# yanxian-ll/GS-SR

Measured on AMD Instinct MI355X. Metric: train iters/sec @300k Gaussians 1080p (rasterize fwd+bwd ms and HBM GB/s vs roofline alongside), higher is better.
Workload: dtype f32; 1 GPU; diff_surfel_rasterization forward+backward (2DGS surfel: the rasterizer of configs[1] scaffold-2dgs) + fused L1/linear image loss + fused Adam (gsrast.optim, one HIP kernel) on EXPLICIT Gaussians, colors_precomp, P=300000, 1920x1080, synthetic scene SURVEY §8d (seed=rank); the complete methods (decode, SSIM, regularisers, statistics) are timed in method_iteration (--full); variant=surfel, P=300000, W=1920, H=1080, parallelism=1 independent tile(s), 1 per GPU, no collective

## Files before the change

gs-sr_amd/csrc/gsr_api.hip:

```cpp
#include "gsr_common.h"
#include <atomic>
#include <cstdarg>
#include <cstdio>
#include <cstring>
#include <mutex>

int gsr_tile_sort_passes(int T);

static thread_local char g_err[512] = "";
void gsr_set_error(const char* fmt, ...)
{
    va_list ap;
    va_start(ap, fmt);
    vsnprintf(g_err, sizeof(g_err), fmt, ap);
    va_end(ap);
}
extern "C" const char* gsr_last_error(void) { return g_err; }
extern "C" int32_t gsr_abi_version(void) { return GSR_ABI_VERSION; }

int gsr_check_launch(const char* what, hipStream_t s, bool debug)
{
    hipError_t e = hipGetLastError();
    if (e != hipSuccess) { gsr_set_error("%s: launch failed: %s", what, hipGetErrorString(e)); return 1; }
    if (debug) {
// ... 54 lines not shown
        else { (void)hipEventCreate(&r.a); (void)hipEventCreate(&r.b); }
        r.label = label;
        (void)hipEventRecord(r.a, s);
    }
    ~ProfScope()
    {
        if (!on) return;
        (void)hipEventRecord(r.b, s);
        std::lock_guard<std::mutex> lk(g_prof_mu);
        g_prof.push_back(r);
    }
};
extern "C" int gsr_profile_enable(int32_t enable)
{
    std::lock_guard<std::mutex> lk(g_prof_mu);
    prof_drain();
    const uint32_t mask = ((uint32_t)enable >> 8) & 0xFFu;
    g_prof_on = enable == 0 ? 0u : ((enable == 1 || mask == 0u) ? 0xFFu : mask);
    for (int i = 0; i < GSR_PROF_LABELS; i++) { g_prof_ms[i] = 0; g_prof_n[i] = 0; }
    return 0;
}
extern "C" int gsr_profile_read(double* ms_total, uint64_t* counts)
{
    std::lock_guard<std::mutex> lk(g_prof_mu);
    prof_drain();
    for (int i = 0; i < GSR_PROF_LABELS; i++) { ms_total[i] = g_prof_ms[i]; counts[i] = g_prof_n[i]; }
    return 0;
}

template <typename T>
static T* take(char*& p, size_t n)
{
    T* r = reinterpret_cast<T*>(p);
    p += gsr_align(n * sizeof(T));
    return r;
}

GeomView gsr_carve_geom(int variant, int P, void* base)
{
    GeomView g;
    char* p = reinterpret_cast<char*>(base);
    const size_t n = (size_t)(P > 0 ? P : 1);
    const uint32_t nblk = gsr_div_up((uint32_t)n, GSR_SORT_BLOCK);
    g.depth_key = take<uint32_t>(p, n);
    g.tiles_touched = take<uint32_t>(p, n);
    g.rect = take<ushort4>(p, n);
    g.cull = take<float4>(p, n * 2);
    g.rec = take<float4>(p, n * gsr_rec_stride(variant));
    g.clamped = take<uint32_t>(p, n);
    g.vals_a = take<uint32_t>(p, n);
    g.offsets = take<uint32_t>(p, n);
    g.keys_b = take<uint32_t>(p, n);
    g.vals_b = take<uint32_t>(p, n);
    g.sorted_idx = g.vals_a;
    g.hist = take<uint32_t>(p, gsr_sort_hist_words(nblk, 256));
    g.scan_tmp = take<uint32_t>(p, gsr_div_up((uint32_t)n, 256) + 64);
    g.counters = take<uint32_t>(p, 64);
    g.bytes = (size_t)(p - reinterpret_cast<char*>(base));
    return g;
}

BinView gsr_carve_bin(int variant, uint32_t R, int W, int H, void* base)
{
    (void)variant;
    BinView b;
    char* p = reinterpret_cast<char*>(base);
    const size_t n = R > 0 ? R : 1;
    const uint32_t nblk = gsr_div_up((uint32_t)n, GSR_SORT_BLOCK);
    b.point_list = take<uint32_t>(p, n);
    b.tile_keys = take<uint32_t>(p, n);
    b.keys_b = take<uint32_t>(p, n);
    b.vals_b = take<uint32_t>(p, n);
    b.hist = take<uint32_t>(p, gsr_sort_hist_words(nblk, 256));
    b.scan_tmp = take<uint32_t>(p, 64);
    {
        const size_t T = (size_t)((W + GSR_TILE - 1) / GSR_TILE) * ((H + GSR_TILE - 1) / GSR_TILE);
        b.qmask = take<unsigned long long>(p, ((n >> 6) + T + 2) * 4);
        b.tile_tab = take<uint32_t>(p, gsr_tile_bucket_words((uint32_t)n, T) + (T <= (size_t)GSR_TB_TILES_MAX ? (size_t)GSR_TB_ROWS_MAX * GSR_TB_GROUPS_MAX : (size_t)2));
    }
    b.cap = R;
    b.bytes = (size_t)(p - reinterpret_cast<char*>(base));
    return b;
}

ImgView gsr_carve_img(int variant, int W, int H, void* base)
{
    ImgView im;
    char* p = reinterpret_cast<char*>(base);
    const size_t N = (size_t)W * H;
    const int gx = (W + GSR_TILE - 1) / GSR_TILE, gy = (H + GSR_TILE - 1) / GSR_TILE;
    im.final_T = take<float>(p, N * (variant == GSR_SURFEL ? 3 : 1));
    im.n_contrib = take<uint32_t>(p, N * (variant == GSR_SURFEL ? 2 : 1));
    im.ranges = take<uint2>(p, (size_t)gx * gy);
    im.tile_order = take<uint32_t>(p, (size_t)gx * gy + 1);
    im.bytes = (size_t)(p - reinterpret_cast<char*>(base));
    return im;
}

extern "C" size_t gsr_geom_bytes(int32_t variant, int32_t P) { return gsr_carve_geom(variant, P, nullptr).bytes; }
extern "C" size_t gsr_img_bytes(int32_t variant, int32_t W, int32_t H) { return gsr_carve_img(variant, W, H, nullptr).bytes; }
extern "C" size_t gsr_binning_bytes(int32_t variant, uint32_t R, int32_t W, int32_t H) { return gsr_carve_bin(variant, R, W, H, nullptr).bytes; }
extern "C" size_t gsr_backward_scratch_bytes(int32_t variant, int32_t P)
{
    return gsr_align((size_t)(P > 0 ? P : 1) * gsr_acc_stride(variant) * sizeof(float));
}

// ... 85 lines not shown
        if (!forced && mb->global_ttl.load(std::memory_order_relaxed) > 0) global = true;
    }
    return global;
}
uint32_t* gsr_long_list_word()
{
    Mailbox* mb = mailbox();
    return mb ? mb->dev + 16 * GSR_MAIL_SLOTS : nullptr;
}

const uint32_t* gsr_static_tile_map(int gx, int gy, hipStream_t s)
{
    struct Ent { int dev, gx, gy; uint32_t* map; };
    static std::mutex mu;
    static std::vector<Ent> cache;
    int dev = 0;
    if (hipGetDevice(&dev) != hipSuccess) return nullptr;
    std::lock_guard<std::mutex> lk(mu);
    for (const Ent& e : cache) if (e.dev == dev && e.gx == gx && e.gy == gy) return e.map;
    {
        hipStreamCaptureStatus cs = hipStreamCaptureStatusNone;
        if (hipStreamIsCapturing(s, &cs) != hipSuccess || cs != hipStreamCaptureStatusNone) { (void)hipGetLastError(); return nullptr; }
    }
    const int T = gx * gy, B = 4, bxn = (gx + B - 1) / B, byn = (gy + B - 1) / B;
    std::vector<std::vector<uint32_t>> lists(8);
    for (int by = 0; by < byn; by++)
        for (int bx = 0; bx < bxn; bx++) {
            std::vector<uint32_t>& L = lists[(bx + 3 * by) & 7];
            for (int ty = by * B; ty < std::min(gy, by * B + B); ty++)
                for (int tx = bx * B; tx < std::min(gx, bx * B + B); tx++) L.push_back((uint32_t)(ty * gx + tx));
        }
    std::vector<uint32_t> map((size_t)T);
    size_t pos[8] = {0, 0, 0, 0, 0, 0, 0, 0};
    for (int b = 0; b < T; b++) {
        int x = b & 7;
        for (int k = 0; k < 8 && pos[x] >= lists[x].size(); k++) x = (x + 1) & 7;
        map[(size_t)b] = lists[x][pos[x]++];
    }
    uint32_t* d = nullptr;
    if (hipMalloc(&d, (size_t)T * sizeof(uint32_t)) != hipSuccess) { (void)hipGetLastError(); return nullptr; }
    if (hipMemcpy(d, map.data(), (size_t)T * sizeof(uint32_t), hipMemcpyHostToDevice) != hipSuccess) { (void)hipGetLastError(); (void)hipFree(d); return nullptr; }
    cache.push_back({dev, gx, gy, d});
    return d;
}

#define GSR_PREFILTERED_MSG "Point is filtered although prefiltered is set. This shouldn't happen!"

static int check_cull_agreement(const gsr_cfg* cfg, const GeomView& g, hipStream_t s)
{
    if (!cfg->debug) return 0;
    uint32_t w = 0u;
    GSR_CHECK(hipMemcpyAsync(&w, g.counters + GSR_CNT_CULL_MISMATCH, sizeof(uint32_t), hipMemcpyDeviceToHost, s), "read cull agreement word");
    GSR_CHECK(hipStreamSynchronize(s), "debug sync");
    if (w) { gsr_set_error("tile culling: k_duplicate emitted a different number of instances than the preprocess kernel counted (gsr_tile_cull.h evaluated differently in the two units)"); return 1; }
    return 0;
}

extern "C" int gsr_forward_stage1_ex(const gsr_cfg* cfg, const gsr_inputs* in, void* geom, size_t geom_bytes,
                                     int32_t* radii, uint32_t* num_rendered_host, uint32_t* depth_order_host, void* stream)
{
    if (check_cfg(cfg, in)) return 1;
    hipStream_t s = (hipStream_t)stream;
    *num_rendered_host = 0;
    if (depth_order_host) *depth_order_host = 0u;
    if (cfg->P == 0) return 0;
    GeomView g = gsr_carve_geom(cfg->variant, cfg->P, geom);
    if (g.bytes > geom_bytes) { gsr_set_error("geom buffer too small: %zu < %zu", geom_bytes, g.bytes); return 1; }
    Mailbox* mb = mailbox();
    const unsigned slot = mb ? take_slot(mb) : 0u;
    struct SlotGuard { Mailbox* m; unsigned s; ~SlotGuard() { if (m) release_slot(m, s); } } guard{mb, slot};
    if (mb) mb->host[16 * slot + 1] = 0u;
    const bool global_order = gsr_decide_depth_order(cfg);
    if (depth_order_host) *depth_order_host = global_order ? GSR_MODE_GLOBAL : GSR_MODE_TILE;
    { ProfScope ps(GSR_PROF_PREPROCESS, s); if (gsr_launch_preprocess(cfg, in, g, radii, s, global_order, mb ? mb->dev + 16 * slot + 1 : nullptr)) return 1; }
    { ProfScope ps(GSR_PROF_DEPTH_ORDER, s); if (gsr_launch_depth_order(cfg, g, mb ? mb->dev + 16 * slot : nullptr, s, global_order, true)) return 1; }
    if (mb) {
        GSR_CHECK(hipStreamSynchronize(s), "stage1 sync");
        *num_rendered_host = *(volatile uint32_t*)(mb->host + 16 * slot);
        if (cfg->prefiltered && *(volatile uint32_t*)(mb->host + 16 * slot + 1)) { gsr_set_error("%s", GSR_PREFILTERED_MSG); return 1; }
    } else {
        GSR_CHECK(hipMemcpyAsync(num_rendered_host, g.counters, sizeof(uint32_t), hipMemcpyDeviceToHost, s), "read num_rendered");
        GSR_CHECK(hipStreamSynchronize(s), "stage1 sync");
    }
    return 0;
}
extern "C" int gsr_forward_stage1(const gsr_cfg* cfg, const gsr_inputs* in, void* geom, size_t geom_bytes,
                                  int32_t* radii, uint32_t* num_rendered_host, void* stream)
{
    return gsr_forward_stage1_ex(cfg, in, geom, geom_bytes, radii, num_rendered_host, nullptr, stream);
}

extern "C" int gsr_forward_stage2_ex(const gsr_cfg* cfg, const gsr_inputs* in, void* geom, size_t geom_bytes,
                                     void* binning, size_t binning_bytes, void* img, size_t img_bytes,
                                     uint32_t num_rendered, uint32_t depth_order, const gsr_outputs* out, void* stream)
{
    if (check_cfg(cfg, in)) return 1;
    hipStream_t s = (hipStream_t)stream;
    (void)geom_bytes;
    GeomView g = gsr_carve_geom(cfg->variant, cfg->P, geom);
    const uint32_t cap = gsr_binning_capacity(cfg->variant, binning_bytes, cfg->W, cfg->H);
    if (cap < num_rendered) { gsr_set_error("binning buffer too small: holds %u instances, need %u", cap, num_rendered); return 1; }
    BinView b = gsr_carve_bin(cfg->variant, cap, cfg->W, cfg->H, binning);
    ImgView im = gsr_carve_img(cfg->variant, cfg->W, cfg->H, img);
    if (im.bytes > img_bytes) { gsr_set_error("img buffer too small: %zu < %zu", img_bytes, im.bytes); return 1; }
    if (cfg->P == 0) {
        return 0;
    }
// ... 199 lines not shown
```

gs-sr_amd/csrc/gsr_binning.hip:

```cpp
#include "gsr_common.h"
#include "gsr_tile_sort.h"
#include "gsr_tile_cull.h"
#include <cstdlib>

__device__ __forceinline__ uint32_t lane_id() { return __builtin_amdgcn_mbcnt_hi(~0u, __builtin_amdgcn_mbcnt_lo(~0u, 0u)); }
__device__ __forceinline__ uint64_t lanemask_lt() { return (1ull << lane_id()) - 1ull; }

__device__ __forceinline__ uint32_t wave_incl_scan(uint32_t v)
{
#pragma unroll
    for (int d = 1; d < 64; d <<= 1) {
        uint32_t t = __shfl_up(v, d, 64);
        if ((int)lane_id() >= d) v += t;
    }
    return v;
}

__device__ __forceinline__ uint32_t block_incl_scan(uint32_t v, uint32_t* lds , uint32_t* total)
{
    const uint32_t lane = threadIdx.x & 63, wave = threadIdx.x >> 6, nw = (blockDim.x + 63) >> 6;
    uint32_t s = wave_incl_scan(v);
    if (lane == 63) lds[wave] = s;
    __syncthreads();
    if (wave == 0) {
// ... 251 lines not shown
        if (dm) hipLaunchKernelGGL(k_scan_rows, dim3(mask + 1), dim3(256), 0, s, H, nblk, gh);
        if (big_blocks) hipLaunchKernelGGL((k_radix_scatter<16, 256>), g, b, 0, s, kin, vin, kout, vout, n, n_dev, shift, bits, H, gh, ngroups, gh_next, dm);
        else hipLaunchKernelGGL((k_radix_scatter<GSR_SORT_ITEMS, 256>), g, b, 0, s, kin, vin, kout, vout, n, n_dev, shift, bits, H, gh, ngroups, gh_next, dm);
        uint32_t* t;
        t = kin; kin = kout; kout = t;
        if (vin == nullptr) { vin = vout; vout = vals_a; }
        else { t = vin; vin = vout; vout = t; }
        in_b = !in_b;
        shift += bits;
    }
    if (result_in_b) *result_in_b = in_b;
    return 0;
}


__global__ void __launch_bounds__(GSR_SCAN_BLOCK) k_offsets_local(const uint32_t* __restrict__ sorted_idx, const uint32_t* __restrict__ tiles_touched,
                                                                  uint32_t P, uint32_t* __restrict__ offsets, uint32_t* __restrict__ block_sums)
{
    __shared__ uint32_t lds[17];
    const uint32_t i = blockIdx.x * GSR_SCAN_BLOCK + threadIdx.x;
    uint32_t v = (i < P) ? tiles_touched[sorted_idx ? sorted_idx[i] : i] : 0;
    uint32_t tot;
    uint32_t incl = block_incl_scan(v, lds, &tot);
    if (i < P) offsets[i] = incl;
    if (threadIdx.x == 0) block_sums[blockIdx.x] = tot;
}
bool gsr_depth_order_static_rule(int P, int T, bool* forced, int variant)
{
    static int mode = -1;
    if (mode < 0) { const char* e = getenv("GSR_DEPTH_ORDER"); mode = !e ? 0 : (e[0] == 'g' ? 1 : (e[0] == 't' ? 2 : 0)); }
    if (forced) *forced = mode != 0;
    if (mode == 1) return true;
    if (mode == 2) return false;
    const long long per_tile = variant == GSR_EWA ? 155ll : (variant == GSR_PLANE ? 176ll : 192ll);
    return (long long)P > per_tile * (long long)T;
}

int gsr_launch_depth_order(const gsr_cfg* cfg, GeomView g, uint32_t* host_word_dev, hipStream_t s, bool global_order, bool need_total)
{
    const uint32_t P = (uint32_t)cfg->P;
    if (!global_order) {
        if (need_total)
            hipLaunchKernelGGL(k_scan_small, dim3(1), dim3(GSR_SCAN_BLOCK), 0, s, g.scan_tmp, gsr_div_up(P, 256u), g.counters, host_word_dev, 1);
        return gsr_check_launch("depth_order", s, cfg->debug);
    }
    bool in_b = false;
    if (gsr_radix_sort_pairs(g.depth_key, g.vals_a, g.keys_b, g.vals_b, P, nullptr, 0, 32, 8, true, g.hist, &in_b, s, false, true)) return 1;
    const uint32_t nblk = gsr_div_up(P, GSR_SCAN_BLOCK);
    hipLaunchKernelGGL(k_offsets_local, dim3(nblk), dim3(GSR_SCAN_BLOCK), 0, s, g.sorted_idx, g.tiles_touched, P, g.offsets, g.scan_tmp);
    hipLaunchKernelGGL(k_scan_small, dim3(1), dim3(GSR_SCAN_BLOCK), 0, s, g.scan_tmp, nblk, g.counters, host_word_dev);
    return gsr_check_launch("depth_order", s, cfg->debug);
}

template <int CULLV>
__global__ void __launch_bounds__(256) k_duplicate(uint32_t P, const uint32_t* __restrict__ sorted_idx, const uint32_t* __restrict__ offsets,
                                                   const uint32_t* __restrict__ block_prefix, const uint32_t* __restrict__ tiles_touched,
                                                   const ushort4* __restrict__ rect, const float4* __restrict__ cull, int gx,
                                                   uint32_t* __restrict__ keys, uint32_t* __restrict__ vals, uint32_t cap,
                                                   uint2* __restrict__ ranges, uint32_t T, uint32_t* __restrict__ zero_ptr, uint32_t zero_n,
                                                   uint32_t* __restrict__ order_valid, uint32_t scan_block,
                                                   uint32_t self_nblk, uint32_t* __restrict__ total_out, uint32_t* __restrict__ host_word)
{
    const uint32_t lane = threadIdx.x & 63u;
    const uint32_t i = (blockIdx.x * blockDim.x + threadIdx.x);
    if (i < T) ranges[i] = make_uint2(0xFFFFFFFFu, 0u);
    for (uint32_t z = i; z < zero_n; z += gridDim.x * blockDim.x) zero_ptr[z] = 0u;
    if (i == 0) *order_valid = 0u;
    const bool v = i < P;
    const uint32_t g = v ? (sorted_idx ? sorted_idx[i] : i) : 0u;
    const uint32_t cnt = v ? tiles_touched[g] : 0u;
    uint32_t bp = 0u;
    if (self_nblk) {
        __shared__ uint32_t s_red[4];
        if (blockIdx.x < self_nblk) {
            uint32_t part = 0u;
            for (uint32_t j = threadIdx.x; j < blockIdx.x; j += 256u) part += block_prefix[j];
#pragma unroll
            for (int d = 32; d >= 1; d >>= 1) part += (uint32_t)__shfl_xor((int)part, d, 64);
            if (lane == 0) s_red[threadIdx.x >> 6] = part;
            __syncthreads();
            bp = (s_red[0] + s_red[1]) + (s_red[2] + s_red[3]);
            if (blockIdx.x == self_nblk - 1u && threadIdx.x == 0) {
                const uint32_t tot = bp + block_prefix[blockIdx.x];
                *total_out = tot;
                if (host_word) __hip_atomic_store(host_word, tot, __ATOMIC_RELAXED, __HIP_MEMORY_SCOPE_SYSTEM);
            }
        }
    } else if (v) bp = block_prefix[i / scan_block];
    const uint32_t incl = v ? offsets[i] + bp : 0u;
    ushort4 r = make_ushort4(0, 0, 1, 1);
    if (cnt) r = rect[g];
    const uint32_t wave_base = __shfl(incl - cnt, 0, 64);
    if constexpr (CULLV >= 0) {
        __shared__ float4 s_cull[2 * 256];
        __shared__ float2 s_slope[256];
        __shared__ ushort4 s_rect[256];
        const uint32_t wbase = threadIdx.x & ~63u;
        float4 c0 = make_float4(0.f, 0.f, 0.f, 0.f), c1 = make_float4(0.f, -1.f, 0.f, 0.f);
        if (cnt) { c0 = cull[2 * (size_t)g]; c1 = cull[2 * (size_t)g + 1]; }
        s_cull[2 * threadIdx.x] = c0; s_cull[2 * threadIdx.x + 1] = c1; s_slope[threadIdx.x] = tc_slopes(c0, c1); s_rect[threadIdx.x] = r;
        __builtin_amdgcn_fence(__ATOMIC_ACQ_REL, "wavefront");
        __builtin_amdgcn_wave_barrier();
        const uint32_t area = cnt ? ((uint32_t)r.z - (uint32_t)r.x) * ((uint32_t)r.w - (uint32_t)r.y) : 0u;
        const uint32_t ai = wave_incl_scan(area);
        const uint32_t total = (uint32_t)__shfl((int)ai, 63, 64), excl = ai - area;
        uint32_t run = wave_base;
        for (uint32_t k0 = 0; k0 < total; k0 += 64u) {
            const TcCand c = tc_candidate<CULLV>(k0 + lane, total, excl, s_cull + 2 * wbase, s_slope + wbase, s_rect + wbase);
            const uint64_t hits = __ballot(c.hit);
            const uint32_t off = run + (uint32_t)__popcll(hits & lanemask_lt());
            const uint32_t sg = (uint32_t)__shfl((int)g, (int)c.s, 64);
            if (c.hit && off < cap) {
                keys[off] = c.ty * (uint32_t)gx + c.tx;
                vals[off] = sg;
            }
            run += (uint32_t)__popcll(hits);
        }
        const uint32_t counted = (uint32_t)__shfl((int)wave_incl_scan(cnt), 63, 64);
        if (lane == 0 && run - wave_base != counted) total_out[GSR_CNT_CULL_MISMATCH] = 1u;
        return;
    }
    uint32_t last = __shfl(incl, 63, 64);
    {
        const uint64_t vm = __ballot(v);
        if (vm != ~0ull) last = vm ? __shfl(incl, 63 - __builtin_clzll(vm), 64) : wave_base;
    }
    const uint32_t total = last - wave_base;
    const uint32_t excl = v ? (incl - cnt) - wave_base : total;
    const uint32_t w = (uint32_t)r.z - (uint32_t)r.x;
    const float rw = 1.0f / (float)(w ? w : 1u);
    for (uint32_t k0 = 0; k0 < total; k0 += 64u) {
        const uint32_t k = k0 + lane;
        uint32_t s = 0;
#pragma unroll
        for (uint32_t step = 32; step >= 1; step >>= 1) {
            const uint32_t t = s + step;
            const uint32_t e = __shfl(excl, t & 63u, 64);
            if (t < 64u && e <= k) s = t;
        }
        const uint32_t j = k - __shfl(excl, s, 64);
        const uint32_t sw = __shfl(w, s, 64), sx0 = __shfl((uint32_t)r.x, s, 64), sy0 = __shfl((uint32_t)r.y, s, 64), sg = __shfl(g, s, 64);
        const float srw = __shfl(rw, s, 64);
        const uint32_t q = (uint32_t)(((float)j + 0.5f) * srw);
        const uint32_t tx = sx0 + (j - q * sw), ty = sy0 + q;
        const uint32_t off = wave_base + k;
        if (k < total && off < cap) {
            keys[off] = ty * (uint32_t)gx + tx;
            vals[off] = sg;
        }
    }
}

__global__ void __launch_bounds__(256) k_tile_ranges(uint32_t R, const uint32_t* __restrict__ n_dev, const uint32_t* __restrict__ tile_keys, uint2* __restrict__ ranges)
{
    if (n_dev) R = min(R, *n_dev);
    const uint32_t i = blockIdx.x * blockDim.x + threadIdx.x;
    if (i >= R) return;
    const uint32_t cur = tile_keys[i];
    if (i == 0) ranges[cur].x = 0;
    else {
        const uint32_t prev = tile_keys[i - 1];
        if (cur != prev) { ranges[prev].y = i; ranges[cur].x = i; }
    }
    if (i == R - 1) ranges[cur].y = R;
}

template <int TH>
__global__ void __launch_bounds__(TH) k_tb_hist(const uint32_t* __restrict__ keys, uint32_t R, const uint32_t* __restrict__ n_dev, uint32_t Tp,
                                                uint32_t* __restrict__ tab, uint32_t* __restrict__ group_prefix)
{
    extern __shared__ uint32_t tb_lds[];
    __shared__ uint32_t gs[GSR_TB_GROUPS_MAX];
// ... 274 lines not shown
    return on != 0;
}

uint32_t gsr_tile_bucket_chunk(bool global_order, int T, uint32_t cap)
{
    static int on = -1;
    if (on < 0) { const char* e = getenv("GSR_TILE_BUCKET"); on = e ? (atoi(e) != 0) : 1; }
    if (!on || global_order || T > GSR_TB_TILES_MAX) return 0u;
    for (uint32_t chunk = 4096u; chunk <= 16384u; chunk <<= 1)
        if (gsr_div_up(cap > 0u ? cap : 1u, chunk) <= GSR_TB_ROWS_MAX) return chunk;
    return 0u;
}

bool gsr_tile_sort_is_fused()
{
    static int fused = -1;
    if (fused < 0) { const char* e = getenv("GSR_TILE_SORT"); fused = (e && e[0] == 'k') ? 0 : 1; }
    return fused != 0;
}

static int tile_bits(int T)
{
    int b = 1;
    while ((1 << b) < T) b++;
    return b;
}
int gsr_tile_sort_passes(int T) { return (tile_bits(T) + 7) / 8; }

int gsr_launch_binning(const gsr_cfg* cfg, GeomView g, BinView b, ImgView im, uint32_t R, const uint32_t* n_dev, hipStream_t s,
                       bool global_order, uint32_t* host_word_dev)
{
    const int gx = (cfg->W + GSR_TILE - 1) / GSR_TILE, gy = (cfg->H + GSR_TILE - 1) / GSR_TILE;
    const int T = gx * gy;
    if (R == 0) {
        const size_t span = (size_t)(reinterpret_cast<char*>(im.tile_order + T + 1) - reinterpret_cast<char*>(im.ranges));
        if (gsr_memset_async(im.ranges, 0, (span + 3) & ~(size_t)3, s)) { gsr_set_error("memset ranges"); return 1; }
        return 0;
    }
    const int passes = gsr_tile_sort_passes(T);
    uint32_t *k0 = (passes & 1) ? b.keys_b : b.tile_keys, *v0 = (passes & 1) ? b.vals_b : b.point_list;
    uint32_t *k1 = (passes & 1) ? b.tile_keys : b.keys_b, *v1 = (passes & 1) ? b.point_list : b.vals_b;
    const uint32_t big_from0 = 1700000u;
    const uint32_t big_from = n_dev ? big_from0 + big_from0 / 4 : big_from0;
    const uint32_t chunk = gsr_tile_bucket_chunk(global_order, T, b.cap);
    const bool bucket = chunk != 0u;
    if (bucket) { k0 = b.keys_b; v0 = b.vals_b; }
    {
        const dim3 dg(gsr_div_up((uint32_t)max(cfg->P, T), 256)), db(256);
        const uint32_t* sidx = global_order ? (const uint32_t*)g.sorted_idx : (const uint32_t*)nullptr;
        const uint32_t zn = bucket ? 0u : gsr_sort_group_words(R, R >= big_from, 256);
        uint32_t* zp = b.hist;
        const uint32_t sblk = global_order ? (uint32_t)GSR_SCAN_BLOCK : 256u;
        const uint32_t snb = global_order ? 0u : gsr_div_up((uint32_t)cfg->P, 256u);
#define GSR_DUP(CV) hipLaunchKernelGGL(k_duplicate<CV>, dg, db, 0, s, (uint32_t)cfg->P, sidx, g.offsets, g.scan_tmp, g.tiles_touched, g.rect, g.cull, gx, k0, v0, R, \
                                       im.ranges, (uint32_t)T, zp, zn, im.tile_order + T, sblk, snb, g.counters, host_word_dev)
        if (!gsr_tile_cull_enabled()) GSR_DUP(-1);
        else if (cfg->variant == GSR_SURFEL) GSR_DUP(GSR_SURFEL);
        else GSR_DUP(GSR_EWA);
#undef GSR_DUP
    }
    if (bucket) {
        const uint32_t rows = gsr_div_up(R, chunk), Tp = ((uint32_t)T + 1u) & ~1u;
        const size_t lds_h = (size_t)(((Tp >> 1) + 31u) & ~31u) * 4u;
        uint32_t* group_prefix = b.tile_tab + gsr_tile_bucket_words(b.cap, (size_t)T);
#define GSR_TB(TH) do { \
        hipLaunchKernelGGL((k_tb_hist<TH>), dim3(rows), dim3(TH), lds_h, s, k0, R, n_dev, Tp, b.tile_tab, group_prefix); \
        hipLaunchKernelGGL(k_tb_columns, dim3(gsr_div_up((uint32_t)T, 64u)), dim3(256), 0, s, b.tile_tab, rows, Tp, (uint32_t)T, group_prefix, im.ranges); \
        hipLaunchKernelGGL((k_tb_scatter<TH>), dim3(rows), dim3(TH), lds_h, s, k0, v0, R, n_dev, Tp, b.tile_tab, b.point_list); } while (0)
        if (chunk == 4096u) GSR_TB(256); else if (chunk == 8192u) GSR_TB(512); else GSR_TB(1024);
#undef GSR_TB
        if (!gsr_tile_sort_is_fused())
            hipLaunchKernelGGL(k_tile_depth_sort, dim3(gsr_div_up((uint32_t)T, 4u)), dim3(256), 0, s, im.ranges, (uint32_t)T, R, g.depth_key, b.point_list, b.tile_keys,
                               b.keys_b, b.vals_b, 1);
        if (gsr_tile_order_wanted()) hipLaunchKernelGGL(k_tile_order, dim3(1), dim3(1024), 0, s, im.ranges, (uint32_t)T, im.tile_order);
        return gsr_check_launch("binning", s, cfg->debug);
    }
    bool in_b = false;
    if (gsr_radix_sort_pairs(k0, v0, k1, v1, R, n_dev, 0, tile_bits(T), 8, false, b.hist, &in_b, s, R >= big_from, true)) return 1;
    hipLaunchKernelGGL(k_tile_ranges, dim3(gsr_div_up(R, 256)), dim3(256), 0, s, R, n_dev, b.tile_keys, im.ranges);
    if (!global_order && !gsr_tile_sort_is_fused())
        hipLaunchKernelGGL(k_tile_depth_sort, dim3(gsr_div_up((uint32_t)T, 4u)), dim3(256), 0, s, im.ranges, (uint32_t)T, R, g.depth_key, b.point_list, b.tile_keys,
                           b.keys_b, b.vals_b, 0);
    if (gsr_tile_order_wanted()) hipLaunchKernelGGL(k_tile_order, dim3(1), dim3(1024), 0, s, im.ranges, (uint32_t)T, im.tile_order);
    return gsr_check_launch("binning", s, cfg->debug);
}
```

gs-sr_amd/csrc/gsr_common.h:

```cpp
#pragma once
#include <hip/hip_runtime.h>
#include <stdint.h>
#include <stddef.h>
#include "../../include/gsrast.h"

#define GSR_TILE 16
#define GSR_WAVE 64
#define GSR_SUB 8

#define GSR_REC_EWA 3
#define GSR_REC_PLANE 4
#define GSR_REC_SURFEL 5
#ifndef GSR_ACC_EWA
#define GSR_ACC_EWA 12
#endif
#define GSR_ACC_PLANE 16
#ifndef GSR_ACC_SURFEL
#define GSR_ACC_SURFEL 20
#endif
#define GSR_ACC_USED_EWA 12
#define GSR_ACC_USED_PLANE 16
#define GSR_ACC_USED_SURFEL 20

#define GSR_SORT_THREADS 256
#define GSR_SORT_ITEMS 4
#define GSR_SORT_BLOCK (GSR_SORT_THREADS * GSR_SORT_ITEMS)
#define GSR_SCAN_BLOCK 1024

static inline __host__ __device__ int gsr_rec_stride(int variant)
{
    return variant == GSR_EWA ? GSR_REC_EWA : (variant == GSR_PLANE ? GSR_REC_PLANE : GSR_REC_SURFEL);
}
static inline __host__ __device__ int gsr_acc_stride(int variant)
{
    return variant == GSR_EWA ? GSR_ACC_EWA : (variant == GSR_PLANE ? GSR_ACC_PLANE : GSR_ACC_SURFEL);
}

static inline __host__ __device__ size_t gsr_align(size_t x, size_t a = 256) { return (x + a - 1) / a * a; }
static inline __host__ __device__ uint32_t gsr_div_up(uint32_t a, uint32_t b) { return (a + b - 1) / b; }

struct GeomView {
    uint32_t* depth_key;
    uint32_t* tiles_touched;
    ushort4* rect;
    float4* cull;
    float4* rec;
    uint32_t* clamped;
    uint32_t* sorted_idx;
    uint32_t* offsets;
    uint32_t* keys_b;
    uint32_t* vals_a;
    uint32_t* vals_b;
    uint32_t* hist;
    uint32_t* scan_tmp;
    uint32_t* counters;
    size_t bytes;
};
struct BinView {
    uint32_t* point_list;
    uint32_t* tile_keys;
    uint32_t* keys_b;
    uint32_t* vals_b;
    uint32_t* hist;
    uint32_t* scan_tmp;
    uint32_t* tile_tab;
    uint32_t cap;
    unsigned long long* qmask;
    size_t bytes;
};
struct ImgView {
    float* final_T;
    uint32_t* n_contrib;
    uint2* ranges;
    uint32_t* tile_order;
    size_t bytes;
};

GeomView gsr_carve_geom(int variant, int P, void* base);
BinView gsr_carve_bin(int variant, uint32_t R, int W, int H, void* base);
ImgView gsr_carve_img(int variant, int W, int H, void* base);

void gsr_set_error(const char* fmt, ...);
int gsr_check_launch(const char* what, hipStream_t s, bool debug);
#define GSR_CHECK(call, what)                                                                \
    do {                                                                                     \
        hipError_t e_ = (call);                                                              \
        if (e_ != hipSuccess) { gsr_set_error("%s: %s", what, hipGetErrorString(e_)); return 1; } \
    } while (0)

#define GSR_CNT_MODE 1
#define GSR_CNT_CULL_MISMATCH 2
#define GSR_MODE_TILE 0x47530001u
#define GSR_MODE_GLOBAL 0x47530002u
bool gsr_decide_depth_order(const gsr_cfg* cfg);
int gsr_launch_preprocess(const gsr_cfg* cfg, const gsr_inputs* in, GeomView g, int32_t* radii, hipStream_t s, bool global_order, uint32_t* prefiltered_err = nullptr);
int gsr_launch_depth_order(const gsr_cfg* cfg, GeomView g, uint32_t* host_word_dev, hipStream_t s, bool global_order, bool need_total);
int gsr_launch_binning(const gsr_cfg* cfg, GeomView g, BinView b, ImgView im, uint32_t R, const uint32_t* n_dev, hipStream_t s,
                       bool global_order, uint32_t* host_word_dev = nullptr);
int gsr_launch_blend_fwd(const gsr_cfg* cfg, const gsr_inputs* in, GeomView g, BinView b, ImgView im,
                         const gsr_outputs* out, hipStream_t s, bool global_order, uint32_t* status_dev = nullptr, uint32_t status_cap = 0u);
int gsr_launch_blend_bwd(const gsr_cfg* cfg, const gsr_inputs* in, GeomView g, BinView b, ImgView im,
                         const gsr_out_grads* og, float* acc, hipStream_t s);
bool gsr_blend_bwd_is_sp();
void gsr_blend_bwd_attach_events(hipEvent_t start, hipEvent_t stop);
bool gsr_depth_order_static_rule(int P, int T, bool* forced, int variant = GSR_SURFEL);
// ... 30 lines not shown
```

gs-sr_amd/csrc/gsr_preprocess.hip:

```cpp
#include "gsr_common.h"
#include "gsr_tile_sort.h"
#include "gsr_tile_cull.h"
#include <stdlib.h>
#include "gsr_math.h"

using namespace gsr;

struct PreParams {
    int P, D, M, W, H, gx, gy, variant;
    float tanfovx, tanfovy, fx, fy, mod;
    const float *means3D, *shs, *colors, *opac, *scales, *rots, *cov3D_pre, *all_map, *view, *proj, *campos;
    int32_t* radii;
    GeomView g;
    const uint8_t* in_mask;
    int scale_stride;
    int no_cull;
    uint32_t* zero_ptr; uint32_t zero_n;
    uint32_t* scan_offsets; uint32_t* scan_sums;
    uint32_t* prefiltered_err;
    uint32_t* mode_word; uint32_t mode;
    int tile_cull;
};
struct PreTc { uint32_t tiles; ushort4 rect; float4 c0, c1; };

__device__ __forceinline__ void load16(const float* p, float* m)
{
#pragma unroll
    for (int i = 0; i < 16; i++) m[i] = p[i];
}

__device__ __forceinline__ float two_tau(float o)
{
    float v = 255.0f * o;
    if (!(v > 1.0f)) return -1.0f;
    return 2.0f * logf(v) * 1.001f + 1e-3f;
}

template <bool FILTER_ONLY>
__device__ __forceinline__ PreTc pre_ewa_one(const PreParams& p, const int idx, const float* sh_staged = nullptr)
{
    PreTc tc; tc.tiles = 0u; tc.rect = make_ushort4(0, 0, 0, 0); tc.c0 = make_float4(0, 0, 0, 0); tc.c1 = make_float4(0, -1, 0, 0);
    if (FILTER_ONLY && p.in_mask && !p.in_mask[idx]) { p.radii[idx] = 0; return tc; }
    float view[16], proj[16];
    load16(p.view, view); load16(p.proj, proj);

    int radius_out = 0; uint32_t tiles = 0, key = 0xFFFFFFFFu, clamped = 0;
    int x0 = 0, y0 = 0, x1 = 0, y1 = 0;
    float4 q0 = make_float4(0, 0, 0, 0), q1 = q0, q2 = q0, q3 = q0, cull0 = q0, cull1 = make_float4(0, -1, 0, 0);

    const float3 p_orig = make_float3(p.means3D[3 * idx], p.means3D[3 * idx + 1], p.means3D[3 * idx + 2]);
    const float3 p_view = xform_point4x3(p_orig, view);
    do {
        if (p_view.z <= 0.2f) {
            if (p.prefiltered_err) __hip_atomic_store(p.prefiltered_err, 1u, __ATOMIC_RELAXED, __HIP_MEMORY_SCOPE_SYSTEM);
            break;
        }
        float4 p_hom = xform_point4x4(p_orig, proj);
        float p_w = 1.0f / (p_hom.w + 0.0000001f);
        float projx = p_hom.x * p_w, projy = p_hom.y * p_w;
        float cov3D[6];
        if (p.cov3D_pre) {
#pragma unroll
            for (int i = 0; i < 6; i++) cov3D[i] = p.cov3D_pre[6 * idx + i];
        } else {
            cov3d_from_scale_rot(p.scales + (size_t)p.scale_stride * idx, p.mod, p.rots + 4 * idx, cov3D);
        }
        Cov2D cv = cov2d_project(p_orig, p.fx, p.fy, p.tanfovx, p.tanfovy, cov3D, view);
        float det = (cv.a * cv.c - cv.b * cv.b);
        if (det == 0.0f) break;
        float det_inv = 1.f / det;
        float conA = cv.c * det_inv, conB = -cv.b * det_inv, conC = cv.a * det_inv;
        float mid = 0.5f * (cv.a + cv.c);
        float lambda1 = mid + sqrtf(fmaxf(0.1f, mid * mid - det));
        float lambda2 = mid - sqrtf(fmaxf(0.1f, mid * mid - det));
// ... 8 lines not shown
        if (p.colors) rgb = make_float3(p.colors[3 * idx], p.colors[3 * idx + 1], p.colors[3 * idx + 2]);
        else rgb = sh_to_rgb(p.D, sh_staged ? sh_staged : p.shs + (size_t)idx * p.M * 3, p_orig,
                             make_float3(p.campos[0], p.campos[1], p.campos[2]), clamped);
        const float o = p.opac[idx];
        key = __float_as_uint(p_view.z);
        tiles = (uint32_t)((y1 - y0) * (x1 - x0));
        q0 = make_float4(pix, piy, conA, conB);
        q1 = make_float4(conC, o, rgb.x, rgb.y);
        q2.x = rgb.z;
        if (p.variant == GSR_PLANE && p.all_map) {
            const float* am = p.all_map + 5 * idx;
            q2.y = am[0]; q2.z = am[1]; q2.w = am[2]; q3.x = am[3]; q3.y = am[4];
        }
        cull0 = make_float4(pix, piy, conA, conB);
        cull1 = make_float4(conC, two_tau(o), 0.f, 0.f);
        {
            const float D = 1.5f * my_radius + 8.f;
            if (!(conA > 0.f && conC > 0.f && conA * conC - conB * conB > 0.f) || !((conA + 2.f * fabsf(conB) + conC) * D * D < 2.5e4f)) {
                cull0.z = 0.f; cull0.w = 0.f; cull1.x = 0.f; if (!(cull1.y > 0.f)) cull1.y = -1.f;
            }
        }
        if (p.no_cull) { cull0 = make_float4(pix, piy, 0.f, 0.f); cull1 = make_float4(0.f, 1.0f, 0.f, 0.f); }
    } while (0);

    p.radii[idx] = radius_out;
    if (FILTER_ONLY) return tc;
    p.g.depth_key[idx] = key;
    tc.tiles = tiles; tc.rect = make_ushort4((unsigned short)x0, (unsigned short)y0, (unsigned short)x1, (unsigned short)y1); tc.c0 = cull0; tc.c1 = cull1;
    p.g.rect[idx] = tc.rect;
    p.g.cull[2 * (size_t)idx] = cull0;
    p.g.cull[2 * (size_t)idx + 1] = cull1;
    p.g.clamped[idx] = clamped;
    const int st = (p.variant == GSR_PLANE) ? GSR_REC_PLANE : GSR_REC_EWA;
    float4* rec = p.g.rec + (size_t)idx * st;
    rec[0] = q0; rec[1] = q1; rec[2] = q2;
    if (p.variant == GSR_PLANE) rec[3] = q3;
    return tc;
}
template <int V>
__device__ __forceinline__ uint32_t pre_tile_count(const PreParams& p, const int idx, const PreTc& tc)
{
    uint32_t tiles = tc.tiles;
    if (p.tile_cull) {
        __shared__ float4 s_cull[2 * 256];
        __shared__ float2 s_slope[256];
        __shared__ ushort4 s_rect[256];
        const uint32_t lane = tds_lane(), wbase = threadIdx.x & ~63u;
        s_cull[2 * threadIdx.x] = tc.c0; s_cull[2 * threadIdx.x + 1] = tc.c1; s_slope[threadIdx.x] = tc_slopes(tc.c0, tc.c1); s_rect[threadIdx.x] = tc.rect;
        __builtin_amdgcn_fence(__ATOMIC_ACQ_REL, "wavefront");
        __builtin_amdgcn_wave_barrier();
        const uint32_t incl = tds_wave_incl_scan(tc.tiles);
        const uint32_t total = (uint32_t)__shfl((int)incl, 63, 64), excl = incl - tc.tiles;
        uint32_t kept = 0u;
        for (uint32_t k0 = 0; k0 < total; k0 += 64u) {
            const TcCand c = tc_candidate<V>(k0 + lane, total, excl, s_cull + 2 * wbase, s_slope + wbase, s_rect + wbase);
            const uint64_t hits = __ballot(c.hit);
            const uint32_t lo = max(excl, k0) - k0, hi = min(incl, k0 + 64u) > k0 ? min(incl, k0 + 64u) - k0 : 0u;
            if (hi > lo) {
                const uint64_t span = (hi >= 64u ? ~0ull : ((1ull << hi) - 1ull)) & ~((1ull << lo) - 1ull);
                kept += (uint32_t)__popcll(hits & span);
            }
        }
        tiles = kept;
    }
    if (idx < p.P) p.g.tiles_touched[idx] = tiles;
    return tiles;
}
__device__ __forceinline__ void pre_block_scan(const PreParams& p, const int idx, const uint32_t tiles)
{
    if (!p.scan_offsets) return;
    __shared__ uint32_t lds[17];
    uint32_t tot;
    const uint32_t incl = tds_block_incl_scan(tiles, lds, &tot);
    if (idx < p.P) p.scan_offsets[idx] = incl;
    if (threadIdx.x == 0) p.scan_sums[blockIdx.x] = tot;
}
template <bool FILTER_ONLY>
__global__ void __launch_bounds__(256) k_preprocess_ewa(PreParams p)
{
    if (p.mode_word && blockIdx.x == 0 && threadIdx.x == 0) { *p.mode_word = p.mode; p.mode_word[GSR_CNT_CULL_MISMATCH - GSR_CNT_MODE] = 0u; }
    for (uint32_t z = (uint32_t)(blockIdx.x * blockDim.x + threadIdx.x); z < p.zero_n; z += gridDim.x * blockDim.x) p.zero_ptr[z] = 0u;
    const int idx = blockIdx.x * blockDim.x + threadIdx.x;
    PreTc tc; tc.tiles = 0u; tc.rect = make_ushort4(0, 0, 0, 0); tc.c0 = make_float4(0, 0, 0, 0); tc.c1 = make_float4(0, -1, 0, 0);
    if (idx < p.P) tc = pre_ewa_one<FILTER_ONLY>(p, idx);
    if (!FILTER_ONLY) pre_block_scan(p, idx, pre_tile_count<GSR_EWA>(p, idx, tc));
}

#define GSR_SH_ROW 49
__device__ __forceinline__ void sh_rows_load(float* my, const float* __restrict__ shs, size_t g0, int lane, size_t total)
{
#pragma unroll
    for (int i = 0; i < 12; i++) {
        const int w = 4 * (i * 64 + lane);
        if (g0 * 48 + w + 3 < total) {
            const float4 v = *reinterpret_cast<const float4*>(shs + g0 * 48 + w);
            const int g = w / 48, j = w - g * 48;
            float* d = my + g * GSR_SH_ROW + j;
            d[0] = v.x; d[1] = v.y; d[2] = v.z; d[3] = v.w;
        }
    }
    __builtin_amdgcn_fence(__ATOMIC_ACQ_REL, "wavefront");
    __builtin_amdgcn_wave_barrier();
}
__device__ __forceinline__ void sh_rows_store(const float* my, float* __restrict__ dst, size_t g0, int lane, size_t total)
{
    __builtin_amdgcn_fence(__ATOMIC_ACQ_REL, "wavefront");
    __builtin_amdgcn_wave_barrier();
#pragma unroll
    for (int i = 0; i < 12; i++) {
        const int w = 4 * (i * 64 + lane);
        if (g0 * 48 + w + 3 < total) {
            const int g = w / 48, j = w - g * 48;
            const float* r = my + g * GSR_SH_ROW + j;
            *reinterpret_cast<float4*>(dst + g0 * 48 + w) = make_float4(r[0], r[1], r[2], r[3]);
        }
    }
// ... 103 lines not shown
    rec[3] = make_float4(normal.x, normal.y, normal.z, rgb.x);
    const double detT = (double)T[0] * ((double)T[4] * T[8] - (double)T[5] * T[7]) - (double)T[1] * ((double)T[3] * T[8] - (double)T[5] * T[6])
                        + (double)T[2] * ((double)T[3] * T[7] - (double)T[4] * T[6]);
    rec[4] = make_float4(rgb.y, rgb.z, (float)detT, 0.f);
    return tc;
}
template <bool SH16>
__global__ void __launch_bounds__(256) k_preprocess_surfel(PreParams p)
{
    if (p.mode_word && blockIdx.x == 0 && threadIdx.x == 0) { *p.mode_word = p.mode; p.mode_word[GSR_CNT_CULL_MISMATCH - GSR_CNT_MODE] = 0u; }
    for (uint32_t z = (uint32_t)(blockIdx.x * blockDim.x + threadIdx.x); z < p.zero_n; z += gridDim.x * blockDim.x) p.zero_ptr[z] = 0u;
    const int idx = blockIdx.x * blockDim.x + threadIdx.x;
    const float* sh_row = nullptr;
    if constexpr (SH16) {
        __shared__ float s_sh[4 * 64 * GSR_SH_ROW];
        const int lane = threadIdx.x & 63;
        float* my = s_sh + (threadIdx.x >> 6) * 64 * GSR_SH_ROW;
        sh_rows_load(my, p.shs, (size_t)(idx - lane), lane, (size_t)p.P * 48);
        sh_row = my + lane * GSR_SH_ROW;
    }
    PreTc tc; tc.tiles = 0u; tc.rect = make_ushort4(0, 0, 0, 0); tc.c0 = make_float4(0, 0, 0, 0); tc.c1 = make_float4(0, -1, 0, 0);
    if (idx < p.P) tc = pre_surfel_one(p, idx, sh_row);
    pre_block_scan(p, idx, pre_tile_count<GSR_SURFEL>(p, idx, tc));
}

__global__ void k_mark_visible(int P, const float* means3D, const float* viewp, uint8_t* present)
{
    const int idx = blockIdx.x * blockDim.x + threadIdx.x;
    if (idx >= P) return;
    float view[16]; load16(viewp, view);
    float3 pv = xform_point4x3(make_float3(means3D[3 * idx], means3D[3 * idx + 1], means3D[3 * idx + 2]), view);
    present[idx] = !(pv.z <= 0.2f);
}

static PreParams make_params(const gsr_cfg* cfg, const gsr_inputs* in, GeomView g, int32_t* radii)
{
    PreParams p;
    p.P = cfg->P; p.D = cfg->D; p.M = cfg->M; p.W = cfg->W; p.H = cfg->H;
    p.gx = (cfg->W + GSR_TILE - 1) / GSR_TILE; p.gy = (cfg->H + GSR_TILE - 1) / GSR_TILE;
    p.variant = cfg->variant;
    p.tanfovx = cfg->tanfovx; p.tanfovy = cfg->tanfovy;
    p.fy = cfg->H / (2.0f * cfg->tanfovy);
    p.fx = cfg->W / (2.0f * cfg->tanfovx);
    p.mod = cfg->scale_modifier;
    p.means3D = in->means3D; p.shs = in->shs; p.colors = in->colors_precomp; p.opac = in->opacities;
    p.scales = in->scales; p.rots = in->rotations; p.cov3D_pre = in->cov3D_precomp; p.all_map = in->all_map;
    p.view = cfg->viewmatrix; p.proj = cfg->projmatrix; p.campos = cfg->campos;
    { const char* e = getenv("GSR_NO_CULL"); p.no_cull = (e && atoi(e) != 0) ? 1 : 0; }
    p.in_mask = nullptr; p.scale_stride = 3;
    p.scan_offsets = nullptr; p.scan_sums = nullptr; p.prefiltered_err = nullptr; p.mode_word = nullptr; p.mode = 0u;
    p.tile_cull = gsr_tile_cull_enabled() ? 1 : 0;
    p.radii = radii; p.g = g;
    p.zero_ptr = nullptr; p.zero_n = 0;
    return p;
}

int gsr_launch_preprocess(const gsr_cfg* cfg, const gsr_inputs* in, GeomView g, int32_t* radii, hipStream_t s, bool global_order, uint32_t* prefiltered_err)
{
    PreParams p = make_params(cfg, in, g, radii);
    p.prefiltered_err = cfg->prefiltered ? prefiltered_err : nullptr;
    p.zero_ptr = g.hist; p.zero_n = global_order ? gsr_sort_group_words((uint32_t)cfg->P, false, 256) : 0u;
    p.mode_word = g.counters + GSR_CNT_MODE; p.mode = global_order ? GSR_MODE_GLOBAL : GSR_MODE_TILE;
    if (!global_order) { p.scan_offsets = g.offsets; p.scan_sums = g.scan_tmp; }
    dim3 grid(gsr_div_up(cfg->P, 256)), block(256);
    const bool sh16 = p.shs && !p.colors && cfg->M == 16 && (((uintptr_t)p.shs) & 15) == 0;
    if (cfg->variant == GSR_SURFEL) { if (sh16) hipLaunchKernelGGL(k_preprocess_surfel<true>, grid, block, 0, s, p); else hipLaunchKernelGGL(k_preprocess_surfel<false>, grid, block, 0, s, p); }
    else if (sh16) hipLaunchKernelGGL(k_preprocess_ewa_sh16, grid, block, 0, s, p);
    else hipLaunchKernelGGL(k_preprocess_ewa<false>, grid, block, 0, s, p);
    return gsr_check_launch("preprocess", s, cfg->debug);
}

extern "C" int gsr_visible_filter(const gsr_cfg* cfg, const float* means3D, const float* scales, const float* rotations,
                                  const float* cov3D_precomp, int32_t* radii, void* stream)
{
    if (cfg->P == 0) return 0;
    gsr_inputs in = {};
    in.means3D = means3D; in.scales = scales; in.rotations = rotations; in.cov3D_precomp = cov3D_precomp;
    GeomView g = {};
    gsr_cfg c = *cfg; c.variant = GSR_EWA;
    PreParams p = make_params(&c, &in, g, radii);
    hipLaunchKernelGGL(k_preprocess_ewa<true>, dim3(gsr_div_up(cfg->P, 256)), dim3(256), 0, (hipStream_t)stream, p);
    return gsr_check_launch("visible_filter", (hipStream_t)stream, cfg->debug);
}

struct LodArgs {
    int Na; const float* anchor; const int32_t* level; const float* extra_level; const float* campos;
    gsr_lod_cfg c;
    uint8_t* anchor_mask; float* prog_ratio; uint8_t* transition_mask;
};
__global__ void __launch_bounds__(256) k_lod_mask(LodArgs p)
{
    const int i = blockIdx.x * blockDim.x + threadIdx.x;
    if (i >= p.Na) return;
    const int lvl = p.level[i];
    const float half = (p.c.voxel_size / 2) / powf(p.c.fork, (float)lvl);
    const float dx = (p.anchor[3 * i] + half) - p.campos[0], dy = (p.anchor[3 * i + 1] + half) - p.campos[1],
                dz = (p.anchor[3 * i + 2] + half) - p.campos[2];
    const float dist = sqrtf(dx * dx + dy * dy + dz * dz) * p.c.resolution_scale;
    float pred = log2f(p.c.standard_dist / dist) / log2f(p.c.fork) + (p.extra_level ? p.extra_level[i] : 0.0f);
    const int cur = p.c.coarse_index - 1;
    int il;
    if (p.c.mode == 3) {
        pred = fminf(fmaxf(pred + 1.0f, 0.9999f), (float)cur + 0.9999f);
        il = (int)floorf(pred);
        if (p.prog_ratio) p.prog_ratio[i] = pred - truncf(pred);
        if (p.transition_mask) p.transition_mask[i] = (lvl == il) ? 1 : 0;
    } else {
        const float r = p.c.mode == 0 ? floorf(pred) : (p.c.mode == 1 ? rintf(pred) : ceilf(pred));
        il = (int)r;
        il = il < 0 ? 0 : (il > cur ? cur : il);
    }
    p.anchor_mask[i] = (lvl <= il) ? 1 : 0;
}

extern "C" int gsr_octree_visible(const gsr_cfg* cfg, const gsr_lod_cfg* lod, const float* anchor, const int32_t* level,
                                  const float* extra_level, const float* scales, int32_t scale_stride, const float* rotations,
// ... 379 lines not shown
```

Baseline: 1385 iters/s.

## Record per-Gaussian tile hit masks in preprocess and replay them in duplicate

In tile-order mode, the preprocess kernel now saves a 64-bit mask of which candidate tiles in each Gaussian's rect passed the cull test. It stores the mask in the otherwise-idle sort scratch buffers. k_duplicate then expands those masks directly with a per-lane binary search and nth-set-bit lookup, instead of re-running the tile-cull test. Gaussians whose rect area exceeds 64 still fall back to the original walk. This avoids a second evaluation of the cull geometry, at the cost of two extra words written and read per Gaussian, plus added shuffle-heavy index math.

```diff
diff --git a/gs-sr_amd/csrc/gsr_api.hip b/gs-sr_amd/csrc/gsr_api.hip
--- a/gs-sr_amd/csrc/gsr_api.hip
+++ b/gs-sr_amd/csrc/gsr_api.hip
@@ -130,6 +130,8 @@
     g.offsets = take<uint32_t>(p, n);
     g.keys_b = take<uint32_t>(p, n);
     g.vals_b = take<uint32_t>(p, n);
+    g.hit_lo = g.keys_b;
+    g.hit_hi = g.vals_b;
     g.sorted_idx = g.vals_a;
     g.hist = take<uint32_t>(p, gsr_sort_hist_words(nblk, 256));
     g.scan_tmp = take<uint32_t>(p, gsr_div_up((uint32_t)n, 256) + 64);
@@ -321,7 +323,7 @@
     uint32_t w = 0u;
     GSR_CHECK(hipMemcpyAsync(&w, g.counters + GSR_CNT_CULL_MISMATCH, sizeof(uint32_t), hipMemcpyDeviceToHost, s), "read cull agreement word");
     GSR_CHECK(hipStreamSynchronize(s), "debug sync");
-    if (w) { gsr_set_error("tile culling: k_duplicate emitted a different number of instances than the preprocess kernel counted (gsr_tile_cull.h evaluated differently in the two units)"); return 1; }
+    if (w) { gsr_set_error("tile culling: k_duplicate emitted a different number of instances than the preprocess kernel counted (a hit mask, or a second walk of gsr_tile_cull.h's test, disagrees with tiles_touched)"); return 1; }
     return 0;
 }
 
diff --git a/gs-sr_amd/csrc/gsr_binning.hip b/gs-sr_amd/csrc/gsr_binning.hip
--- a/gs-sr_amd/csrc/gsr_binning.hip
+++ b/gs-sr_amd/csrc/gsr_binning.hip
@@ -327,10 +327,22 @@
     return gsr_check_launch("depth_order", s, cfg->debug);
 }
 
+__device__ __forceinline__ uint32_t nth_set_bit(uint64_t m, uint32_t j)
+{
+    uint32_t pos = 0u, x = (uint32_t)m, c = (uint32_t)__popc(x);
+    if (j >= c) { j -= c; pos = 32u; x = (uint32_t)(m >> 32); }
+#pragma unroll
+    for (uint32_t h = 16u; h >= 1u; h >>= 1) {
+        c = (uint32_t)__popc(x & ((1u << h) - 1u));
+        if (j >= c) { j -= c; pos += h; x >>= h; }
+    }
+    return pos;
+}
 template <int CULLV>
 __global__ void __launch_bounds__(256) k_duplicate(uint32_t P, const uint32_t* __restrict__ sorted_idx, const uint32_t* __restrict__ offsets,
                                                    const uint32_t* __restrict__ block_prefix, const uint32_t* __restrict__ tiles_touched,
-                                                   const ushort4* __restrict__ rect, const float4* __restrict__ cull, int gx,
+                                                   const ushort4* __restrict__ rect, const float4* __restrict__ cull,
+                                                   const uint32_t* __restrict__ hit_lo, const uint32_t* __restrict__ hit_hi, int gx,
                                                    uint32_t* __restrict__ keys, uint32_t* __restrict__ vals, uint32_t cap,
                                                    uint2* __restrict__ ranges, uint32_t T, uint32_t* __restrict__ zero_ptr, uint32_t zero_n,
                                                    uint32_t* __restrict__ order_valid, uint32_t scan_block,
@@ -367,32 +379,74 @@
     if (cnt) r = rect[g];
     const uint32_t wave_base = __shfl(incl - cnt, 0, 64);
     if constexpr (CULLV >= 0) {
-        __shared__ float4 s_cull[2 * 256];
-        __shared__ float2 s_slope[256];
-        __shared__ ushort4 s_rect[256];
-        const uint32_t wbase = threadIdx.x & ~63u;
-        float4 c0 = make_float4(0.f, 0.f, 0.f, 0.f), c1 = make_float4(0.f, -1.f, 0.f, 0.f);
-        if (cnt) { c0 = cull[2 * (size_t)g]; c1 = cull[2 * (size_t)g + 1]; }
-        s_cull[2 * threadIdx.x] = c0; s_cull[2 * threadIdx.x + 1] = c1; s_slope[threadIdx.x] = tc_slopes(c0, c1); s_rect[threadIdx.x] = r;
-        __builtin_amdgcn_fence(__ATOMIC_ACQ_REL, "wavefront");
-        __builtin_amdgcn_wave_barrier();
         const uint32_t area = cnt ? ((uint32_t)r.z - (uint32_t)r.x) * ((uint32_t)r.w - (uint32_t)r.y) : 0u;
-        const uint32_t ai = wave_incl_scan(area);
-        const uint32_t total = (uint32_t)__shfl((int)ai, 63, 64), excl = ai - area;
-        uint32_t run = wave_base;
-        for (uint32_t k0 = 0; k0 < total; k0 += 64u) {
-            const TcCand c = tc_candidate<CULLV>(k0 + lane, total, excl, s_cull + 2 * wbase, s_slope + wbase, s_rect + wbase);
-            const uint64_t hits = __ballot(c.hit);
-            const uint32_t off = run + (uint32_t)__popcll(hits & lanemask_lt());
-            const uint32_t sg = (uint32_t)__shfl((int)g, (int)c.s, 64);
-            if (c.hit && off < cap) {
-                keys[off] = c.ty * (uint32_t)gx + c.tx;
-                vals[off] = sg;
+        const uint32_t first = incl - cnt;
+        const bool walk = cnt && (!hit_lo || area > 64u);
+        bool bad = false;
+        if (hit_lo) {
+            uint64_t m = 0ull;
+            if (cnt && !walk) m = (uint64_t)hit_lo[g] | ((uint64_t)hit_hi[g] << 32);
+            const uint32_t mc = walk ? 0u : cnt;
+            bad = mc && (uint32_t)__popcll(m) != mc;
+            const uint32_t mi = wave_incl_scan(mc);
+            const uint32_t mtotal = (uint32_t)__shfl((int)mi, 63, 64), mex = mi - mc;
+            const uint32_t w = (uint32_t)r.z - (uint32_t)r.x;
+            const float rw = 1.0f / (float)(w ? w : 1u);
+            for (uint32_t k0 = 0; k0 < mtotal; k0 += 64u) {
+                const uint32_t k = k0 + lane;
+                uint32_t s = 0;
+#pragma unroll
+                for (uint32_t step = 32; step >= 1; step >>= 1) {
+                    const uint32_t t = s + step;
+                    const uint32_t e = __shfl(mex, t & 63u, 64);
+                    if (t < 64u && e <= k) s = t;
+                }
+                const uint32_t j = k - __shfl(mex, s, 64);
+                const uint64_t sm = ((uint64_t)__shfl((uint32_t)(m >> 32), s, 64) << 32) | (uint64_t)__shfl((uint32_t)m, s, 64);
+                const uint32_t c = nth_set_bit(sm, j);
+                const uint32_t sw = __shfl(w, s, 64), sx0 = __shfl((uint32_t)r.x, s, 64), sy0 = __shfl((uint32_t)r.y, s, 64);
+                const uint32_t sg = __shfl(g, s, 64), sf = __shfl(first, s, 64);
+                const float srw = __shfl(rw, s, 64);
+                const uint32_t q = (uint32_t)(((float)c + 0.5f) * srw);
+                const uint32_t off = sf + j;
+                if (k < mtotal && off < cap) {
+                    keys[off] = (sy0 + q) * (uint32_t)gx + sx0 + (c - q * sw);
+                    vals[off] = sg;
+                }
             }
-            run += (uint32_t)__popcll(hits);
-        }
-        const uint32_t counted = (uint32_t)__shfl((int)wave_incl_scan(cnt), 63, 64);
-        if (lane == 0 && run - wave_base != counted) total_out[GSR_CNT_CULL_MISMATCH] = 1u;
+        }
+        if (__ballot(walk) != 0ull) {
+            __shared__ float4 s_cull[2 * 256];
+            __shared__ float2 s_slope[256];
+            __shared__ ushort4 s_rect[256];
+            const uint32_t wbase = threadIdx.x & ~63u;
+            float4 c0 = make_float4(0.f, 0.f, 0.f, 0.f), c1 = make_float4(0.f, -1.f, 0.f, 0.f);
+            if (walk) { c0 = cull[2 * (size_t)g]; c1 = cull[2 * (size_t)g + 1]; }
+            s_cull[2 * threadIdx.x] = c0; s_cull[2 * threadIdx.x + 1] = c1; s_slope[threadIdx.x] = tc_slopes(c0, c1); s_rect[threadIdx.x] = r;
+            __builtin_amdgcn_fence(__ATOMIC_ACQ_REL, "wavefront");
+            __builtin_amdgcn_wave_barrier();
+            const uint32_t wa = walk ? area : 0u;
+            const uint32_t ai = wave_incl_scan(wa);
+            const uint32_t total = (uint32_t)__shfl((int)ai, 63, 64), excl = ai - wa;
+            uint32_t done = 0u;
+            for (uint32_t k0 = 0; k0 < total; k0 += 64u) {
+                const TcCand c = tc_candidate<CULLV>(k0 + lane, total, excl, s_cull + 2 * wbase, s_slope + wbase, s_rect + wbase);
+                const uint64_t hits = __ballot(c.hit);
+                const uint32_t slo = min(max((uint32_t)__shfl((int)excl, (int)c.s, 64), k0) - k0, 63u);
+                const uint32_t before = (uint32_t)__popcll(hits & lanemask_lt() & ~((1ull << slo) - 1ull));
+                const uint32_t sd = (uint32_t)__shfl((int)done, (int)c.s, 64), sf = (uint32_t)__shfl((int)first, (int)c.s, 64);
+                const uint32_t sg = (uint32_t)__shfl((int)g, (int)c.s, 64);
+                const uint32_t off = sf + sd + before;
+                if (c.hit && off < cap) {
+                    keys[off] = c.ty * (uint32_t)gx + c.tx;
+                    vals[off] = sg;
+                }
+                const uint32_t lo = max(excl, k0) - k0, hi = min(ai, k0 + 64u) > k0 ? min(ai, k0 + 64u) - k0 : 0u;
+                if (hi > lo) done += (uint32_t)__popcll(hits & ((hi >= 64u ? ~0ull : ((1ull << hi) - 1ull)) & ~((1ull << lo) - 1ull)));
+            }
+            bad |= walk && done != cnt;
+        }
+        if (__ballot(bad) != 0ull && lane == 0) total_out[GSR_CNT_CULL_MISMATCH] = 1u;
         return;
     }
     uint32_t last = __shfl(incl, 63, 64);
@@ -773,7 +827,8 @@
         uint32_t* zp = b.hist;
         const uint32_t sblk = global_order ? (uint32_t)GSR_SCAN_BLOCK : 256u;
         const uint32_t snb = global_order ? 0u : gsr_div_up((uint32_t)cfg->P, 256u);
-#define GSR_DUP(CV) hipLaunchKernelGGL(k_duplicate<CV>, dg, db, 0, s, (uint32_t)cfg->P, sidx, g.offsets, g.scan_tmp, g.tiles_touched, g.rect, g.cull, gx, k0, v0, R, \
+#define GSR_DUP(CV) hipLaunchKernelGGL(k_duplicate<CV>, dg, db, 0, s, (uint32_t)cfg->P, sidx, g.offsets, g.scan_tmp, g.tiles_touched, g.rect, g.cull, \
+                                       global_order ? nullptr : g.hit_lo, global_order ? nullptr : g.hit_hi, gx, k0, v0, R, \
                                        im.ranges, (uint32_t)T, zp, zn, im.tile_order + T, sblk, snb, g.counters, host_word_dev)
         if (!gsr_tile_cull_enabled()) GSR_DUP(-1);
         else if (cfg->variant == GSR_SURFEL) GSR_DUP(GSR_SURFEL);
diff --git a/gs-sr_amd/csrc/gsr_common.h b/gs-sr_amd/csrc/gsr_common.h
--- a/gs-sr_amd/csrc/gsr_common.h
+++ b/gs-sr_amd/csrc/gsr_common.h
@@ -51,6 +51,8 @@
     uint32_t* keys_b;
     uint32_t* vals_a;
     uint32_t* vals_b;
+    uint32_t* hit_lo;
+    uint32_t* hit_hi;
     uint32_t* hist;
     uint32_t* scan_tmp;
     uint32_t* counters;
diff --git a/gs-sr_amd/csrc/gsr_preprocess.hip b/gs-sr_amd/csrc/gsr_preprocess.hip
--- a/gs-sr_amd/csrc/gsr_preprocess.hip
+++ b/gs-sr_amd/csrc/gsr_preprocess.hip
@@ -20,6 +20,7 @@
     uint32_t* prefiltered_err;
     uint32_t* mode_word; uint32_t mode;
     int tile_cull;
+    uint32_t* hit_lo; uint32_t* hit_hi;
 };
 struct PreTc { uint32_t tiles; ushort4 rect; float4 c0, c1; };
 
@@ -134,16 +135,21 @@
         const uint32_t incl = tds_wave_incl_scan(tc.tiles);
         const uint32_t total = (uint32_t)__shfl((int)incl, 63, 64), excl = incl - tc.tiles;
         uint32_t kept = 0u;
+        uint64_t mask = 0ull;
         for (uint32_t k0 = 0; k0 < total; k0 += 64u) {
             const TcCand c = tc_candidate<V>(k0 + lane, total, excl, s_cull + 2 * wbase, s_slope + wbase, s_rect + wbase);
             const uint64_t hits = __ballot(c.hit);
             const uint32_t lo = max(excl, k0) - k0, hi = min(incl, k0 + 64u) > k0 ? min(incl, k0 + 64u) - k0 : 0u;
             if (hi > lo) {
                 const uint64_t span = (hi >= 64u ? ~0ull : ((1ull << hi) - 1ull)) & ~((1ull << lo) - 1ull);
-                kept += (uint32_t)__popcll(hits & span);
+                const uint64_t mine = hits & span;
+                kept += (uint32_t)__popcll(mine);
+                const uint32_t c0 = max(excl, k0) - excl;
+                if (c0 < 64u) mask |= (mine >> lo) << c0;
             }
         }
         tiles = kept;
+        if (p.hit_lo && idx < p.P) { p.hit_lo[idx] = (uint32_t)mask; p.hit_hi[idx] = (uint32_t)(mask >> 32); }
     }
     if (idx < p.P) p.g.tiles_touched[idx] = tiles;
     return tiles;
@@ -353,6 +359,7 @@
     p.tile_cull = gsr_tile_cull_enabled() ? 1 : 0;
     p.radii = radii; p.g = g;
     p.zero_ptr = nullptr; p.zero_n = 0;
+    p.hit_lo = nullptr; p.hit_hi = nullptr;
     return p;
 }
 
@@ -362,7 +369,7 @@
     p.prefiltered_err = cfg->prefiltered ? prefiltered_err : nullptr;
     p.zero_ptr = g.hist; p.zero_n = global_order ? gsr_sort_group_words((uint32_t)cfg->P, false, 256) : 0u;
     p.mode_word = g.counters + GSR_CNT_MODE; p.mode = global_order ? GSR_MODE_GLOBAL : GSR_MODE_TILE;
-    if (!global_order) { p.scan_offsets = g.offsets; p.scan_sums = g.scan_tmp; }
+    if (!global_order) { p.scan_offsets = g.offsets; p.scan_sums = g.scan_tmp; p.hit_lo = g.hit_lo; p.hit_hi = g.hit_hi; }
     dim3 grid(gsr_div_up(cfg->P, 256)), block(256);
     const bool sh16 = p.shs && !p.colors && cfg->M == 16 && (((uintptr_t)p.shs) & 15) == 0;
     if (cfg->variant == GSR_SURFEL) { if (sh16) hipLaunchKernelGGL(k_preprocess_surfel<true>, grid, block, 0, s, p); else hipLaunchKernelGGL(k_preprocess_surfel<false>, grid, block, 0, s, p); }
```

Result: no change. 1391 iters/s, median of 6 (+0.5%).
